# rasd3/TODA

Hardware: AMD Instinct MI355X
Metric: LiDAR training samples/sec (higher is better)
Workload: dtype f32

## Files before the change

toda_amd/csrc/rulebook.hip:

```cpp
#include "grid_index.cuh"
#include "scan.cuh"

namespace toda {

constexpr int RB_BLOCK = GI_TILE;

__global__ void __launch_bounds__(RB_BLOCK)
gi_mark_coords_kernel(const int4* __restrict__ idx, int n, const int32_t* __restrict__ n_dev, GridDims g,
                      uint2* __restrict__ cells) {
    n = eff_n(n, n_dev);
    const int i = blockIdx.x * RB_BLOCK + threadIdx.x;
    if (i >= n) return;
    const int4 c = idx[i];
    if (!in_grid(c, g)) return;
    gi_set_bit_first(cells, lin_index(c.x, c.y, c.z, c.w, g));
}

__global__ void __launch_bounds__(RB_BLOCK)
gi_rowof_kernel(const int4* __restrict__ idx, int n, const int32_t* __restrict__ n_dev, GridDims g,
                const uint2* __restrict__ cells, int* __restrict__ rowof) {
    n = eff_n(n, n_dev);
    const int i = blockIdx.x * RB_BLOCK + threadIdx.x;
    if (i >= n) return;
    const int4 c = idx[i];
// ... 332 lines not shown
    pairs_open(s_cnt, K);
    const int i = blockIdx.x * RB_BLOCK + threadIdx.x;
    const bool live = i < n_in;
    int4 c = make_int4(0, 0, 0, 0);
    if (live) c = idx[i];
    const bool inside = live && (unsigned)c.x < (unsigned)cg.out.B;
    int zo[KZ], yo[KY], xo[KX];
#pragma unroll
    for (int a = 0; a < KZ; ++a) zo[a] = out_coord(c.y, a, cg.st[0], cg.pd[0], cg.out.D);
#pragma unroll
    for (int a = 0; a < KY; ++a) yo[a] = out_coord(c.z, a, cg.st[1], cg.pd[1], cg.out.H);
#pragma unroll
    for (int a = 0; a < KX; ++a) xo[a] = out_coord(c.w, a, cg.st[2], cg.pd[2], cg.out.W);
    uint2 cell[K];
    unsigned bit[K];
#pragma unroll
    for (int k = 0; k < K; ++k) {
        const Tap t = tap_of<KY, KX>(k);
        cell[k] = make_uint2(0u, 0u);
        bit[k] = 0u;
        if (inside && zo[t.z] >= 0 && yo[t.y] >= 0 && xo[t.x] >= 0) gi_fetch(cells, lin_index(c.x, zo[t.z], yo[t.y], xo[t.x], cg.out), cell[k], bit[k]);
    }
#pragma unroll
    for (int k = 0; k < K; ++k) {
        int o = gi_rank_of(cell[k], bit[k]);
        if (o >= n_out) o = -1;
        if (o >= 0 && o2i) o2i[(size_t)k * n_out + o] = i;
        if (live) i2o[(size_t)k * n_in + i] = o;
        count_pairs(o >= 0, k, s_cnt);
    }
    pairs_flush(s_cnt, K, pair_cnt);
}

template <int KZ, int KY, int KX>
__global__ void __launch_bounds__(RB_BLOCK)
rb_conv_o2i_kernel(const int4* __restrict__ idx_out, int n_out, ConvGeom cg, GridDims gin, const uint2* __restrict__ cells_in,
                   const int* __restrict__ rowof_in, int n_in, int* __restrict__ o2i) {
    constexpr int K = KZ * KY * KX;
    const int o = blockIdx.x * RB_BLOCK + threadIdx.x;
    if (o >= n_out) return;
    const int4 c = idx_out[o];
    uint2 cell[K];
    unsigned bit[K];
#pragma unroll
    for (int k = 0; k < K; ++k) {
        const Tap t = tap_of<KY, KX>(k);
        cell[k] = make_uint2(0u, 0u);
        bit[k] = 0u;
        const int z = in_coord(c.y, t.z, cg.st[0], cg.pd[0]), y = in_coord(c.z, t.y, cg.st[1], cg.pd[1]), x = in_coord(c.w, t.x, cg.st[2], cg.pd[2]);
        if (in_grid(make_int4(c.x, z, y, x), gin)) gi_fetch(cells_in, lin_index(c.x, z, y, x, gin), cell[k], bit[k]);
    }
    int r[K];
#pragma unroll
    for (int k = 0; k < K; ++k) {
        r[k] = gi_rank_of(cell[k], bit[k]);
        if (r[k] >= n_in) r[k] = -1;
    }
    if (rowof_in) {
#pragma unroll
        for (int k = 0; k < K; ++k)
            if (r[k] >= 0) r[k] = rowof_in[r[k]];
    }
#pragma unroll
    for (int k = 0; k < K; ++k) o2i[(size_t)k * n_out + o] = r[k];
}

// ... 3 lines not shown
    __shared__ int s_cnt[64];
    pairs_open(s_cnt, 64);
    const int i = blockIdx.x * RB_BLOCK + threadIdx.x;
    const bool live = i < n_in;
    int4 c = make_int4(0, 0, 0, 0);
    if (live) c = idx[i];
    const bool inside = live && (unsigned)c.x < (unsigned)cg.out.B;
    int k = 0;
    for (int kz = 0; kz < cg.ks[0]; ++kz) {
        const int zo = out_coord(c.y, kz, cg.st[0], cg.pd[0], cg.out.D);
        for (int ky = 0; ky < cg.ks[1]; ++ky) {
            const int yo = out_coord(c.z, ky, cg.st[1], cg.pd[1], cg.out.H);
            for (int kx = 0; kx < cg.ks[2]; ++kx, ++k) {
                const int xo = out_coord(c.w, kx, cg.st[2], cg.pd[2], cg.out.W);
                uint2 cell = {};
                unsigned bit = 0u;
                if (inside && zo >= 0 && yo >= 0 && xo >= 0) gi_fetch(cells, lin_index(c.x, zo, yo, xo, cg.out), cell, bit);
                int o = gi_rank_of(cell, bit);
                if (o >= n_out) o = -1;
                if (o >= 0) o2i[(size_t)k * n_out + o] = i;
                if (live) i2o[(size_t)k * n_in + i] = o;
                count_pairs(o >= 0, k, s_cnt);
            }
        }
    }
    pairs_flush(s_cnt, k, pair_cnt);
}

struct ConvKernels {
    decltype(&rb_conv_generic_kernel) i2o;
    decltype(&rb_conv_o2i_kernel<3, 3, 3>) o2i;
};

static ConvKernels conv_kernels(const int32_t* ks) {
    if (ks[0] == 3 && ks[1] == 3 && ks[2] == 3) return {rb_conv_kernel<3, 3, 3>, rb_conv_o2i_kernel<3, 3, 3>};
    if (ks[0] == 3 && ks[1] == 1 && ks[2] == 1) return {rb_conv_kernel<3, 1, 1>, rb_conv_o2i_kernel<3, 1, 1>};
    return {rb_conv_generic_kernel, nullptr};
}

static int conv_setup(const char* who, int batch, const int32_t* shape_in, const int32_t* ks, const int32_t* st, const int32_t* pd,
                      const int32_t* shape_out, const void* gi_out, GiView* out, ConvGeom* cg) {
    int rc = gi_view(who, gi_out, batch, shape_out, out);
    if (rc) return rc;
    for (int a = 0; a < 3; ++a) {
        TODA_CHECK_ARG(ks[a] >= 1 && st[a] >= 1 && pd[a] >= 0, "%s: bad kernel/stride/pad on axis %d", who, a);
        TODA_CHECK_ARG(shape_in[a] + 2 * pd[a] >= ks[a], "%s: axis %d of %d cells (+ 2 * %d) is shorter than the kernel's %d", who, a,
                       shape_in[a], pd[a], ks[a]);
        const int expect = (shape_in[a] + 2 * pd[a] - ks[a]) / st[a] + 1;
        TODA_CHECK_ARG(shape_out[a] == expect, "%s: shape_out[%d]=%d but (in+2p-k)/s+1=%d", who, a, shape_out[a], expect);
        cg->ks[a] = ks[a];
        cg->st[a] = st[a];
        cg->pd[a] = pd[a];
    }
    TODA_CHECK_ARG(ks[0] * ks[1] * ks[2] <= 64, "%s: kernel volume > 64 unsupported", who);
    cg->out = out->dims;
    return TODA_OK;
}

}

using namespace toda;

extern "C" size_t toda_gridindex_bytes(int batch, const int32_t* shape_host) {
    return gi_layout(batch, shape_host).bytes;
}

extern "C" int toda_gridindex_from_coords(const int32_t* idx, int n, const int32_t* n_dev, int batch,
                                          const int32_t* shape_host, void* gi, int32_t* rowof, void* stream) {
// ... 101 lines not shown
    GiView v;
    int rc = gi_view("rulebook_subm", gi, batch, shape_host, &v);
    if (rc) return rc;
    const int K = ksize_host[0] * ksize_host[1] * ksize_host[2];
    TODA_CHECK_ARG(K >= 1 && K <= 64, "rulebook_subm: kernel volume %d unsupported", K);
    for (int a = 0; a < 3; ++a)
        TODA_CHECK_ARG(ksize_host[a] % 2 == 1 && dilation_host[a] >= 1, "rulebook_subm: kernel must be odd, dilation >= 1");
    if (!cnt_zeroed) TODA_HIP(hipMemsetAsync(pair_cnt, 0, K * sizeof(int32_t), s));
    if (n == 0) return TODA_OK;
    const uint2* cells = v.cells;
    const dim3 grid(cdiv(n, RB_BLOCK)), block(RB_BLOCK);
    if (ksize_host[0] == 3 && ksize_host[1] == 3 && ksize_host[2] == 3)
        hipLaunchKernelGGL(HIP_KERNEL_NAME(rb_subm_kernel<3, 3, 3>), grid, block, 0, s, (const int4*)idx, n, v.dims,
                           dilation_host[0], dilation_host[1], dilation_host[2], cells, rowof, nbr, pair_cnt);
    else
        hipLaunchKernelGGL(rb_subm_generic_kernel, grid, block, 0, s, (const int4*)idx, n, v.dims, ksize_host[0],
                           ksize_host[1], ksize_host[2], dilation_host[0], dilation_host[1], dilation_host[2], cells,
                           rowof, nbr, pair_cnt);
    TODA_LAUNCH_CHECK();
    return TODA_OK;
}

extern "C" int toda_rulebook_conv(const int32_t* idx_in, int n_in, int batch, const int32_t* shape_in_host,
                                  const int32_t* ksize_host, const int32_t* stride_host, const int32_t* pad_host,
                                  const int32_t* shape_out_host, const void* gi_out, int n_out, int32_t* nbr_o2i,
                                  int32_t* nbr_i2o, int32_t* pair_cnt, const int32_t* idx_out, const void* gi_in,
                                  const int32_t* rowof_in, int cnt_zeroed, void* stream) {
    hipStream_t s = (hipStream_t)stream;
    GiView out;
    ConvGeom cg;
    int rc = conv_setup("rulebook_conv", batch, shape_in_host, ksize_host, stride_host, pad_host, shape_out_host, gi_out, &out, &cg);
    if (rc) return rc;
    const int K = ksize_host[0] * ksize_host[1] * ksize_host[2];
    const ConvKernels kernels = conv_kernels(ksize_host);
    const bool by_output = idx_out && gi_in && kernels.o2i;
    if (!cnt_zeroed) TODA_HIP(hipMemsetAsync(pair_cnt, 0, K * sizeof(int32_t), s));
    if (n_out > 0 && !by_output) TODA_HIP(hipMemsetAsync(nbr_o2i, 0xFF, (size_t)K * n_out * sizeof(int32_t), s));
    const dim3 block(RB_BLOCK);
    if (by_output && n_out > 0) {
        GiView in;
        rc = gi_view("rulebook_conv", gi_in, batch, shape_in_host, &in);
        if (rc) return rc;
        hipLaunchKernelGGL(kernels.o2i, dim3(cdiv(n_out, RB_BLOCK)), block, 0, s, (const int4*)idx_out, n_out, cg, in.dims,
                           (const uint2*)in.cells, rowof_in, n_in, nbr_o2i);
    }
    if (n_in > 0)
        hipLaunchKernelGGL(kernels.i2o, dim3(cdiv(n_in, RB_BLOCK)), block, 0, s, (const int4*)idx_in, n_in, cg, (const uint2*)out.cells,
                           n_out, by_output ? nullptr : nbr_o2i, nbr_i2o, pair_cnt);
    TODA_LAUNCH_CHECK();
    return TODA_OK;
}
```

toda_amd/csrc/spconv.hip:

```cpp
#include <stdlib.h>

#include <type_traits>

#include <hip/hip_ext.h>

#include <mutex>
#include <vector>

#include "bn_fold.cuh"
#include "common.h"


namespace toda {

typedef float f32x4 __attribute__((ext_vector_type(4)));

constexpr int SC_BLOCK = 256;

static int tiles_pow2(int channels) {
    int t = (channels + 15) / 16, p = 1;
    while (p < t) p <<= 1;
    return p;
}

// ... 213 lines not shown
                to = qo[done + lane];
            }
            __builtin_amdgcn_wave_barrier();
            if (lane < left) {
                qi[lane] = ti;
                qo[lane] = to;
            }
        }
        qn = left;
        __builtin_amdgcn_wave_barrier();
    }
    if (qn > 0) round(0, qn, std::false_type{});
}

template <bool BOUND, int MTB, int NTB>
__device__ __forceinline__ void wg_store_slab(const f32x4 (&acc)[MTB][NTB], float* slab, int chunk, int k, int K, int MT, int NT,
                                              int m0, int n0, int cin, int cout, int ii, int g) {
    float* dst = slab + (size_t)chunk * cout * K * cin;
#pragma unroll
    for (int m = 0; m < MTB; ++m)
#pragma unroll
        for (int n = 0; n < NTB; ++n)
#pragma unroll
            for (int reg = 0; reg < 4; ++reg) {
                const int ci = MT * (4 * g + reg) + m0 + m;
                const int co = NT * ii + n0 + n;
                if (!BOUND || (ci < cin && co < cout)) dst[((size_t)co * K + k) * cin + ci] = acc[m][n][reg];
            }
}

struct GatherClasses {
    unsigned char count[8];
    unsigned char k[8][27];
};

template <int Q, int NT, int RT, bool VEC, bool CLS = false>
__global__ void __launch_bounds__(SC_BLOCK)
gather_gemm_kernel(const float* __restrict__ in, int n_in, int cg, const float* __restrict__ wp,
                   const int* __restrict__ nbr, int n_out, int K, int cp, const float* __restrict__ bias,
                   float* __restrict__ out, const int* __restrict__ order,
                   const unsigned char* __restrict__ cls_sorted, const GatherClasses classes) {
    const int lane = threadIdx.x & 63;
    const int wave = (int)blockIdx.x * (SC_BLOCK / 64) + (threadIdx.x >> 6);
    const int r = lane & 15, g = lane >> 4;
    const int row0 = wave * (16 * RT);
    if (row0 >= n_out) return;

    f32x4 acc[RT][NT];
#pragma unroll
    for (int n = 0; n < NT; ++n) {
        float b = 0.0f;
        if (bias && NT * r + n < cp) b = bias[NT * r + n];
#pragma unroll
        for (int rt = 0; rt < RT; ++rt) acc[rt][n] = f32x4{b, b, b, b};
    }
    const f32x4* __restrict__ wp4 = reinterpret_cast<const f32x4*>(wp);
    const __amdgpu_buffer_rsrc_t in_rsrc = table_rsrc(in, (unsigned)n_in * (unsigned)cg * 4u);
    int rows[RT];
    bool live[RT];
#pragma unroll
    for (int rt = 0; rt < RT; ++rt) {
        live[rt] = row0 + rt * 16 + r < n_out;
        rows[rt] = live[rt] ? (order ? order[row0 + rt * 16 + r] : row0 + rt * 16 + r) : n_out - 1;
    }

    auto load_ids = [&](int k, int (&dst)[RT]) {
// ... 731 lines not shown
    for (int s = 0; s < n; ++s) {
        TODA_CHECK_ARG(w[s] && wp[s] && cout[s] >= 1 && cin[s] >= 1 && k_vol[s] >= 1, "pack_weights: bad segment %d", s);
        const int cgather = transpose[s] ? cout[s] : cin[s], cprod = transpose[s] ? cin[s] : cout[s];
        TODA_CHECK_ARG(cgather <= 128 && cprod <= 128, "pack_weights: channels > 128 unsupported (segment %d)", s);
        if (use_split(cgather, cprod)) {
            split_pack_fill(sb, sm, w[s], cout[s], k_vol[s], cin[s], transpose[s], flip_k[s], wp[s]);
            const long long total = (long long)k_vol[s] * sb.KC[sm] * sb.NT[sm] * 192;
            if (total > smost) smost = total;
            if (++sm == toda::SPLIT_PACK_MAX_SEG) {
                const int rc = sflush();
                if (rc != TODA_OK) return rc;
            }
            continue;
        }
        const int i = m;
        b.w[i] = w[s], b.wp[i] = wp[s], b.cout[i] = cout[s], b.K[i] = k_vol[s], b.cin[i] = cin[s];
        b.transpose[i] = transpose[s] != 0, b.flip[i] = flip_k[s] != 0;
        b.Q[i] = (unsigned char)tiles_pow2(cgather), b.NT[i] = (unsigned char)tiles_pow2(cprod);
        const long long total = (long long)k_vol[s] * b.Q[i] * b.NT[i] * 256;
        if (total > most) most = total;
        if (++m == PACK_MAX_SEG) {
            const int rc = flush();
            if (rc != TODA_OK) return rc;
        }
    }
    {
        const int rc = flush();
        if (rc != TODA_OK) return rc;
    }
    return sflush();
}

namespace toda {
constexpr int CLS_ROWS = 8192, CLS_PER = CLS_ROWS / 256;
struct ClassGeom {
    int stride[3], pad[3];
};
__global__ void __launch_bounds__(256)
class_order_kernel(const int4* __restrict__ coords, int n, const ClassGeom gm, int32_t* __restrict__ order, unsigned char* __restrict__ cls_sorted) {
    __shared__ int cnt[8][256 + 1];
    const int base = blockIdx.x * CLS_ROWS, t = threadIdx.x;
    unsigned char c[CLS_PER];
    int mine[8] = {0, 0, 0, 0, 0, 0, 0, 0};
#pragma unroll
    for (int i = 0; i < CLS_PER; ++i) {
        const int r = base + t * CLS_PER + i;
        int cl = 0;
        if (r < n) {
            const int4 v = coords[r];
            cl = (((v.y + gm.pad[0]) % gm.stride[0]) * gm.stride[1] + (v.z + gm.pad[1]) % gm.stride[1]) * gm.stride[2] + (v.w + gm.pad[2]) % gm.stride[2];
            ++mine[cl & 7];
        }
        c[i] = (unsigned char)cl;
    }
#pragma unroll
    for (int k = 0; k < 8; ++k) cnt[k][t] = mine[k];
    __syncthreads();
    if (t < 8) {
        int run = 0;
        for (int j = 0; j < 256; ++j) {
            const int v = cnt[t][j];
            cnt[t][j] = run;
            run += v;
        }
        cnt[t][256] = run;
    }
    __syncthreads();
    int cls_base[8], run = 0;
#pragma unroll
    for (int k = 0; k < 8; ++k) {
        cls_base[k] = run + cnt[k][t];
        run += cnt[k][256];
    }
#pragma unroll
    for (int i = 0; i < CLS_PER; ++i) {
        const int r = base + t * CLS_PER + i;
        if (r >= n) break;
        const int k = c[i] & 7;
        int pos = 0;
#pragma unroll
        for (int q = 0; q < 8; ++q)
            if (q == k) pos = cls_base[q]++;
        order[base + pos] = r;
        cls_sorted[base + pos] = c[i];
    }
}

static int class_table(const int32_t* ksize, const int32_t* stride, const int32_t* pad, GatherClasses* out) {
    const int n_class = stride[0] * stride[1] * stride[2];
    if (n_class < 1 || n_class > 8 || ksize[0] * ksize[1] * ksize[2] > 27) return -1;
    *out = GatherClasses{};
    for (int rz = 0; rz < stride[0]; ++rz)
        for (int ry = 0; ry < stride[1]; ++ry)
            for (int rx = 0; rx < stride[2]; ++rx) {
                const int c = (rz * stride[1] + ry) * stride[2] + rx;
                int m = 0;
                for (int kz = 0; kz < ksize[0]; ++kz)
                    for (int ky = 0; ky < ksize[1]; ++ky)
                        for (int kx = 0; kx < ksize[2]; ++kx)
                            if (kz % stride[0] == rz && ky % stride[1] == ry && kx % stride[2] == rx)
                                out->k[c][m++] = (unsigned char)((kz * ksize[1] + ky) * ksize[2] + kx);
                out->count[c] = (unsigned char)m;
            }
    return 0;
}
}

extern "C" int toda_rulebook_class_order(const int32_t* in_coords, int n_in, const int32_t* stride, const int32_t* padding, int32_t* order,
                                         unsigned char* cls_sorted, void* stream) {
    TODA_CHECK_ARG(in_coords && stride && padding && order && cls_sorted && n_in >= 0, "rulebook_class_order: null argument");
    ClassGeom gm;
    for (int a = 0; a < 3; ++a) {
        TODA_CHECK_ARG(stride[a] >= 1 && stride[a] <= 2 && padding[a] >= 0, "rulebook_class_order: stride 1 or 2 per axis (got %d)", stride[a]);
        gm.stride[a] = stride[a], gm.pad[a] = padding[a];
    }
    if (n_in == 0) return TODA_OK;
    hipLaunchKernelGGL(class_order_kernel, dim3(cdiv(n_in, CLS_ROWS)), dim3(256), 0, (hipStream_t)stream, (const int4*)in_coords, n_in, gm, order,
                       cls_sorted);
    TODA_LAUNCH_CHECK();
    return TODA_OK;
}

namespace toda {
struct LaunchTimer {
    std::vector<hipEvent_t> ev;
    int used = 0;
    bool on = false;
};
static LaunchTimer g_timer;
static std::mutex g_timer_mu;
static inline void timer_next(hipEvent_t* start, hipEvent_t* stop) {
    *start = *stop = nullptr;
    if (!g_timer.on) return;
    std::lock_guard<std::mutex> lock(g_timer_mu);
    if (!g_timer.on || 2 * (g_timer.used + 1) > (int)g_timer.ev.size()) return;
    *start = g_timer.ev[2 * g_timer.used];
    *stop = g_timer.ev[2 * g_timer.used + 1];
    g_timer.used++;
}
}

#define GG_LAUNCH(kernel, grid, block, shmem, stream, ...)                                              \
    do {                                                                                               \
        hipEvent_t t0_, t1_;                                                                           \
        toda::timer_next(&t0_, &t1_);                                                                  \
        hipExtLaunchKernelGGL(kernel, grid, block, shmem, stream, t0_, t1_, 0, __VA_ARGS__);           \
    } while (0)

extern "C" int toda_timing_begin(int capacity) {
    TODA_CHECK_ARG(capacity > 0 && capacity <= (1 << 20), "timing_begin: capacity in (0, 2^20]");
// ... 331 lines not shown
```

toda_amd/csrc/spconv_split.cuh:

```cuda
#pragma once
#include "split_common.cuh"

namespace toda {

#ifndef WGS_ACCS
#define WGS_ACCS 2
#endif
#ifndef SP_STAMPS
#define SP_STAMPS 0
#endif
#if SP_STAMPS
#define SP_STAMP(i)                                                                               \
    do {                                                                                          \
        unsigned long long t_;                                                                    \
        __builtin_amdgcn_sched_barrier(0);                                                        \
        asm volatile("s_memtime %0\n\ts_waitcnt lgkmcnt(0)" : "=s"(t_)::"memory");                \
        __builtin_amdgcn_sched_barrier(0);                                                        \
        seg[i] += t_ - t_prev;                                                                    \
        t_prev = t_;                                                                              \
    } while (0)
#else
#define SP_STAMP(i)
#endif
#ifndef SP_ABLATE
// ... 72 lines not shown
        } else {
            if (gch < cout && pch < cin) x = w[((size_t)gch * K + kk) * cin + pch];
        }
        v[j] = sp_plane_of(x, plane);
    }
    b.wps[sg][e] = u32x4{(unsigned)v[0] | ((unsigned)v[1] << 16), (unsigned)v[2] | ((unsigned)v[3] << 16), (unsigned)v[4] | ((unsigned)v[5] << 16),
                         (unsigned)v[6] | ((unsigned)v[7] << 16)};
}

template <int KC, int NT, int WAVES, bool IL = false>
__global__ void __launch_bounds__(SC_BLOCK, WAVES)
gg_split_kernel(const float* __restrict__ in, int n_in, const u32x4* __restrict__ wps, const int* __restrict__ nbr, int n_out, int K, int cp,
                const float* __restrict__ bias, float* __restrict__ out, const int* __restrict__ order, double* __restrict__ stats,
                const unsigned char* __restrict__ cls_sorted, const GatherClasses classes) {
    constexpr int RT = 2;
    constexpr int CG = 32 * KC;
    constexpr int UNITS = NT * 3;
    constexpr int SLICE = UNITS * 64;
    static_assert(2 * SLICE * 16 >= (SC_BLOCK / 64) * 2 * 16 * NT * 4, "the statistics scratch aliases the weight buffers");
    __shared__ u32x4 wl[2 * SLICE];
    const int lane = threadIdx.x & 63, wv = threadIdx.x >> 6;
    const int blk = xcd_chunked_block(blockIdx.x, gridDim.x);
    const int wave = blk * (SC_BLOCK / 64) + wv;
    const int r = lane & 15, g = lane >> 4;
    const int row0 = wave * (16 * RT);

    f32x4 acc[RT][NT];
    int rows[RT];
    bool live[RT];
    gg_prologue<RT, NT>(bias, cp, row0, n_out, order, r, acc, rows, live);
    const __amdgpu_buffer_rsrc_t in_rsrc = table_rsrc(in, (unsigned)n_in * (unsigned)CG * 4u);
    int KE = K;
    bool listed = false;
    unsigned long long kpack = 0;
    if (cls_sorted) {
        const int p = row0 + (lane & (16 * RT - 1));
        const int c = cls_sorted[p < n_out ? p : n_out - 1], c0 = __builtin_amdgcn_readfirstlane(c);
        const bool same = __all(c == c0 || p >= n_out);
        int* cw = reinterpret_cast<int*>(wl);
        if (lane == 0) cw[wv] = same ? c0 : -1;
        __syncthreads();
        int cb = cw[0];
#pragma unroll
        for (int w = 1; w < SC_BLOCK / 64; ++w) cb = (cw[w] == cb) ? cb : -1;
        __syncthreads();
        if (cb >= 0 && classes.count[cb & 7] > 0 && classes.count[cb & 7] <= 8) {
            listed = true;
            KE = classes.count[cb & 7];
#pragma unroll
            for (int i = 0; i < 8; ++i) kpack |= (unsigned long long)classes.k[cb & 7][i] << (8 * i);
            kpack = ((unsigned long long)__builtin_amdgcn_readfirstlane((int)(kpack >> 32)) << 32) | (unsigned)__builtin_amdgcn_readfirstlane((int)kpack);
        }
    }
    auto kof = [&](int j) { return listed ? (int)((kpack >> (8 * j)) & 0xFF) : j; };
    auto load_ids = [&](int j, int (&dst)[RT]) {
        const int kk = kof(j < KE ? j : KE - 1);
#pragma unroll
        for (int rt = 0; rt < RT; ++rt) {
            dst[rt] = __builtin_nontemporal_load(nbr + (size_t)kk * n_out + rows[rt]);
        }
    };
    auto gather_rt = [&](const int (&src)[RT], int part, bool valid, f32x4 (&raw)[RT][2], int rt) {
        const bool ok = src[rt] >= 0 && valid;
        const unsigned base = (unsigned)src[rt] * (unsigned)(CG * 4) + (unsigned)(16 * g) + 128u * (unsigned)part;
#pragma unroll
        for (int i = 0; i < 2; ++i)
            raw[rt][i] = __builtin_bit_cast(f32x4, __builtin_amdgcn_raw_buffer_load_b128(in_rsrc, ok ? base + 64u * i : OOB, 0, 0));
    };
    auto gather = [&](const int (&src)[RT], int part, bool valid, f32x4 (&raw)[RT][2]) {
#pragma unroll
        for (int rt = 0; rt < RT; ++rt) gather_rt(src, part, valid, raw, rt);
    };
    auto stage = [&](int st, int buf) {
        const int sc = st < KE * KC ? st : KE * KC - 1;
        const int ss = kof(sc / KC) * KC + sc % KC;
#pragma unroll
        for (int t = 0; t < (UNITS + SC_BLOCK / 64 - 1) / (SC_BLOCK / 64); ++t) {
            const int u = t * (SC_BLOCK / 64) + wv;
            if (UNITS % (SC_BLOCK / 64) == 0 || u < UNITS)
                __builtin_amdgcn_global_load_lds(reinterpret_cast<const float*>(wps + (size_t)ss * SLICE + u * 64 + lane),
                                                 reinterpret_cast<float*>(&wl[buf * SLICE + u * 64]), 16, 0, 0);
        }
    };

    int idA[RT], idB[RT], idC[RT];
    f32x4 raw[RT][2];
    load_ids(0, idA);
// ... 286 lines not shown
```

toda_amd/csrc/conv2d.hip:

```cpp
#include <hip/hip_ext.h>
#include <stdlib.h>
#include <string.h>

#include <algorithm>

#include "common.h"

#ifndef TODA_ABLATE
#define TODA_ABLATE 0
#endif

namespace toda {

typedef float f32x4 __attribute__((ext_vector_type(4)));
typedef float f32x2 __attribute__((ext_vector_type(2)));
typedef unsigned int u32x4w __attribute__((ext_vector_type(4)));

constexpr int WN_BLOCK = 256;
constexpr int WN_TILES = 32;
constexpr int WN_COUT = 32;
constexpr int WN_KC = 8;
constexpr int WN_FREQ = 36;
constexpr int WN_IMG = 256;
constexpr unsigned WN_OOB = 0xFFFFFFF0u;
// ... 77 lines not shown

__global__ void __launch_bounds__(WN_BLOCK)
wino_weight_kernel(const float* __restrict__ w, int cout, int cin, int mode, float* __restrict__ u) {
    wn_weight_element(w, cout, cin, mode, u, blockIdx.x * WN_BLOCK + threadIdx.x);
}

constexpr int WB_MAX_LAYERS = 16;
struct WeightBatch {
    const float* w[WB_MAX_LAYERS];
    float* u[WB_MAX_LAYERS];
    int cout[WB_MAX_LAYERS], cin[WB_MAX_LAYERS], mode[WB_MAX_LAYERS];
    unsigned first_block[WB_MAX_LAYERS + 1];
    int n;
};

__global__ void __launch_bounds__(WN_BLOCK)
wino_weight_batch_kernel(const WeightBatch b) {
    int l = 0;
    while (l + 1 < b.n && blockIdx.x >= b.first_block[l + 1]) ++l;
    wn_weight_element(b.w[l], b.cout[l], b.cin[l], b.mode[l], b.u[l], (blockIdx.x - b.first_block[l]) * WN_BLOCK + threadIdx.x);
}

__device__ __forceinline__ __amdgpu_buffer_rsrc_t wn_rsrc(const float* base, unsigned bytes) {
    return __builtin_amdgcn_make_buffer_rsrc(const_cast<float*>(base), 0, bytes, 0x00020000);
}

__device__ __forceinline__ int wn_work_id() {
    const int nwg = gridDim.x, xcd = blockIdx.x & 7, q8 = nwg >> 3, r8 = nwg & 7;
    return (xcd < r8 ? xcd * (q8 + 1) : r8 * (q8 + 1) + (xcd - r8) * q8) + (blockIdx.x >> 3);
}

struct PatchOff {
    unsigned offc[6];
    unsigned offe[6];
    bool left, right;
    bool tail;
};

__device__ __forceinline__ PatchOff wn_patch_off(int tile, int t, int chan, int C, const WinoGeom& g) {
    PatchOff p;
    const bool exists = tile < g.n_tiles;
    const int tl = exists ? tile : 0;
    const int b = tl / g.tiles_img, rem = tl - b * g.tiles_img;
    const int ty = rem / g.tiles_x, tx = rem - ty * g.tiles_x;
    const int y0 = 4 * ty, x0 = 4 * tx;
    const int base = ((b * C + chan) * g.H + (y0 - 1)) * g.W + x0;
    const bool has_l = x0 > 0, has_r = x0 + 4 < g.W;
    p.left = has_l || t == 0;
    p.right = has_r || t == 15;
    p.tail = x0 + 3 >= g.W;
#pragma unroll
    for (int r = 0; r < 6; ++r) {
        const int yy = y0 - 1 + r;
        const bool rv = exists && yy >= 0 && yy < g.H;
        const int row = base + r * g.W;
        p.offc[r] = rv ? (unsigned)row * 4u : WN_OOB;
        p.offe[r] = (rv && t == 0 && has_l) ? (unsigned)(row - 1) * 4u : (rv && t == 15 && has_r) ? (unsigned)(row + 4) * 4u : WN_OOB;
    }
    return p;
}

struct Patch {
    f32x2 p[6], q[6], e[6];
};

__device__ __forceinline__ float wn_dpp_from_prev(float own, float v) {
    return __builtin_bit_cast(float, __builtin_amdgcn_update_dpp(__builtin_bit_cast(int, own), __builtin_bit_cast(int, v), 0x111, 0xF, 0xF, false));
}
__device__ __forceinline__ float wn_dpp_from_next(float own, float v) {
    return __builtin_bit_cast(float, __builtin_amdgcn_update_dpp(__builtin_bit_cast(int, own), __builtin_bit_cast(int, v), 0x101, 0xF, 0xF, false));
}

__device__ __forceinline__ void wn_load_patch(__amdgpu_buffer_rsrc_t rsrc, const PatchOff& o, unsigned soff, Patch& d) {
#pragma unroll
    for (int r = 0; r < 6; ++r) {
        const f32x4 c = __builtin_bit_cast(f32x4, __builtin_amdgcn_raw_buffer_load_b128(rsrc, o.offc[r], soff, 0));
        const float e = __builtin_bit_cast(float, __builtin_amdgcn_raw_buffer_load_b32(rsrc, o.offe[r], soff, 0));
        const float l = wn_dpp_from_prev(e, c[3]), rr = wn_dpp_from_next(e, c[0]);
        d.p[r] = f32x2{c[0], c[1]};
        d.q[r] = f32x2{o.tail ? 0.0f : c[2], o.tail ? 0.0f : c[3]};
        d.e[r] = f32x2{o.left ? l : 0.0f, o.right ? rr : 0.0f};
    }
}

struct PatchRaw {
    f32x4 c[6];
    float e[6];
    bool left, right, tail;
};

__device__ __forceinline__ void wn_load_raw(__amdgpu_buffer_rsrc_t rsrc, const PatchOff& o, unsigned soff, PatchRaw& d) {
#pragma unroll
    for (int r = 0; r < 6; ++r) {
        d.c[r] = __builtin_bit_cast(f32x4, __builtin_amdgcn_raw_buffer_load_b128(rsrc, o.offc[r], soff, 0));
        d.e[r] = __builtin_bit_cast(float, __builtin_amdgcn_raw_buffer_load_b32(rsrc, o.offe[r], soff, 0));
    }
    d.left = o.left, d.right = o.right, d.tail = o.tail;
}

__device__ __forceinline__ void wn_finish_patch(const PatchRaw& s, Patch& d) {
#pragma unroll
    for (int r = 0; r < 6; ++r) {
        const float l = wn_dpp_from_prev(s.e[r], s.c[r][3]), rr = wn_dpp_from_next(s.e[r], s.c[r][0]);
        d.p[r] = f32x2{s.c[r][0], s.c[r][1]};
        d.q[r] = f32x2{s.tail ? 0.0f : s.c[r][2], s.tail ? 0.0f : s.c[r][3]};
        d.e[r] = f32x2{s.left ? l : 0.0f, s.right ? rr : 0.0f};
    }
}

__device__ __forceinline__ f32x2 wn_fma2(float c, f32x2 a, f32x2 b) {
    return __builtin_elementwise_fma(f32x2{c, c}, a, b);
}

__device__ __forceinline__ void wn_bt2(const f32x2 (&d)[6], f32x2 (&v)[6]) {
    const f32x2 a = d[3] - d[1], b = d[4] - d[2];
    v[0] = wn_fma2(1.5f, a, wn_fma2(-2.0f, d[2], d[0] + d[4]));
    v[1] = wn_fma2(-2.5f, d[2], wn_fma2(0.5f, d[3], d[1] + d[4]));
    v[2] = wn_fma2(2.5f, d[3], wn_fma2(0.5f, d[2], d[4] - d[1]));
    v[3] = wn_fma2(2.0f, a, b);
    v[4] = wn_fma2(-0.5f, a, b);
    v[5] = wn_fma2(1.5f, b, wn_fma2(-2.0f, d[3], d[1] + d[5]));
}

__device__ __forceinline__ f32x2 w2_lo(f32x2 a) { return __builtin_shufflevector(a, a, 0, 0); }
__device__ __forceinline__ f32x2 w2_hi(f32x2 a) { return __builtin_shufflevector(a, a, 1, 1); }
__device__ __forceinline__ f32x2 w2_fma(f32x2 a, f32x2 b, f32x2 c) { return __builtin_elementwise_fma(a, b, c); }
#define W2_K(a_, b_) ((unsigned long long)__builtin_bit_cast(unsigned, (float)(a_)) | ((unsigned long long)__builtin_bit_cast(unsigned, (float)(b_)) << 32))
#define W2_KK(a_) W2_K(a_, a_)
__device__ __forceinline__ f32x2 w2_add(f32x2 a, f32x2 b) {
    f32x2 d;
    asm("v_pk_add_f32 %0, %1, %2" : "=v"(d) : "v"(a), "v"(b));
    return d;
}
__device__ __forceinline__ f32x2 w2_sub(f32x2 a, f32x2 b) {
    f32x2 d;
    asm("v_pk_add_f32 %0, %1, %2 neg_lo:[0,1] neg_hi:[0,1]" : "=v"(d) : "v"(a), "v"(b));
    return d;
}
__device__ __forceinline__ f32x2 w2_mul(f32x2 a, f32x2 b) {
    f32x2 d;
// ... 337 lines not shown
                }
            } else if (!(ablate & 4)) wn_input_transform_store(d, lds + buf * IMG + a_off);
            else lds[buf * IMG + a_off] = d.p[0][0] + d.e[5][1] + d.q[2][0];
        };

        WinoCursor ld = ws_cursor(lo, g.n_chunks, true);
        PatchOff pa = patch_of(ld.unit);
        const unsigned x_bytes = (unsigned)((size_t)g.B * g.Cin * g.H * g.W * 4u), u_bytes = (unsigned)((size_t)WN_FREQ * g.Cin * g.Cout * 4u);
        const unsigned u_voff = (unsigned)pt * 16u;
        auto fetch = [&](Stage& st, int q_fetch) {
            const bool live = q_fetch < total;
            const __amdgpu_buffer_rsrc_t xr_q = wn_rsrc(x, live && !(ablate & 1) ? x_bytes : 0u);
            const __amdgpu_buffer_rsrc_t ur_q = wn_rsrc(u, live && !(ablate & 2) ? u_bytes : 0u);
            wn_load_raw(xr_q, pa, (unsigned)ld.chunk * chunk_bytes, st.d);
            const unsigned u_soff = (unsigned)((cb_of(ld.unit) * g.n_chunks + ld.chunk) * IMG) * 4u;
#pragma unroll
            for (int it = 0; it < B_IT; ++it)
                st.b[it] = __builtin_bit_cast(f32x4, __builtin_amdgcn_raw_buffer_load_b128(ur_q, u_voff, u_soff + (unsigned)it * 4096u, 0));
            if (live) {
                if (++ld.chunk == g.n_chunks) {
                    ld.chunk = 0;
                    ld.unit += 1;
                    if (q_fetch + 1 < total && (gang || ld.unit % g.n_cout_blocks == 0)) pa = patch_of(ld.unit);
                }
            }
        };
        wn_produce_stream<Stage>(total, fetch, produce);
    }
}

constexpr int WG_KT = 8;
constexpr int WG_SLAB_FLOATS = WN_FREQ * 32 * 32;

struct TilePos {
    int b, ty, tx;
    bool exists;
};

__device__ __forceinline__ TilePos wn_tile_pos(int tile, const WinoGeom& g) {
    TilePos t;
    t.exists = tile < g.n_tiles;
    const int tl = t.exists ? tile : 0;
    t.b = tl / g.tiles_img;
    const int rem = tl - t.b * g.tiles_img;
    t.ty = rem / g.tiles_x;
    t.tx = rem - t.ty * g.tiles_x;
    return t;
}

__device__ __forceinline__ void wn_tile_advance(TilePos& t, int step, int tile_after, const WinoGeom& g) {
    t.tx += step;
    while (t.tx >= g.tiles_x) {
        t.tx -= g.tiles_x;
        if (++t.ty == g.tiles_y) {
            t.ty = 0;
            ++t.b;
        }
    }
    t.exists = tile_after < g.n_tiles;
}

__device__ __forceinline__ float wn_quad_from_prev(float own, float v) {
    const float s = __builtin_bit_cast(float, __builtin_amdgcn_update_dpp(0, __builtin_bit_cast(int, v), 0x90, 0xF, 0xF, false));
    return (threadIdx.x & 3) == 0 ? own : s;
}
__device__ __forceinline__ float wn_quad_from_next(float own, float v) {
// ... 79 lines not shown
        asm("v_pk_fma_f32 %0, %1, %2, %1 op_sel:[1,0,0] op_sel_hi:[1,1,0]" : "=v"(u) : "v"(P), "s"(W2_K(0.5f, -2.0f)));
        asm("v_pk_fma_f32 %0, %1, %2, %0 op_sel:[0,0,0] op_sel_hi:[0,1,1]" : "+v"(u) : "v"(Q), "s"(W2_K(0.25f, 4.0f)));
        asm("v_pk_fma_f32 %0, %1, %2, %0 op_sel:[1,0,0] op_sel_hi:[1,1,1]" : "+v"(u) : "v"(Q), "s"(W2_K(0.125f, -8.0f)));
        dst[(i * 6 + 0) * WN_IMG] = P[0];
        dst[(i * 6 + 1) * WN_IMG] = m12[0];
        dst[(i * 6 + 2) * WN_IMG] = m12[1];
        dst[(i * 6 + 3) * WN_IMG] = u[0];
        dst[(i * 6 + 4) * WN_IMG] = u[1];
        dst[(i * 6 + 5) * WN_IMG] = Q[1];
    }
}

struct WgradGeom {
    WinoGeom g;
    int n_ci_blocks, n_co_blocks, n_units, steps_per_unit;
};

__global__ void __launch_bounds__(WS_BLOCK, 2)
wino_wgrad_kernel(const float* __restrict__ x, const float* __restrict__ dy, const WgradGeom wg, float* __restrict__ slabs, const int ablate_arg) {
    const int ablate = TODA_ABLATE ? ablate_arg : 0;
    __shared__ float lds[4 * WN_FREQ * WN_IMG];
    constexpr int IMG = WN_FREQ * WN_IMG;
    const WinoGeom& g = wg.g;
    const int tid = threadIdx.x, lane = tid & 63, wave = tid >> 6;
    const int G = gridDim.x;
    const int w = wn_work_id();
    const long long S = (long long)wg.n_units * wg.steps_per_unit;
    const long long lo = ws_range_lo(w, G, S), hi = ws_range_lo(w + 1, G, S);
    const int total = __builtin_amdgcn_readfirstlane((int)(hi - lo));
    if (total == 0) return;

    if (wave < 4) {
        const int wm = wave >> 1, wn = wave & 1;
        const f32x2* const a_frag = reinterpret_cast<const f32x2*>(lds) + wm * 64 + lane;
        const f32x2* const b_frag = reinterpret_cast<const f32x2*>(lds + 2 * IMG) + wn * 64 + lane;
        int q = 0;
        long long s = lo;
        while (s < hi) {
            const WinoCursor at = ws_cursor(s, wg.steps_per_unit);
            const int unit = at.unit, c_begin = at.chunk, c_end = ws_segment_end(s, hi, c_begin, wg.steps_per_unit);
            f32x4 acc[WN_FREQ];
#pragma unroll
            for (int f = 0; f < WN_FREQ; ++f) acc[f] = f32x4{0.f, 0.f, 0.f, 0.f};
            for (int chunk = c_begin; chunk < c_end; ++chunk, ++q) {
                __syncthreads();
                wn_consume_chunk(acc, a_frag + (q & 1) * (IMG / 2), b_frag + (q & 1) * (IMG / 2), ablate);
            }
            s += c_end - c_begin;
            float* const sl = slabs + (size_t)(w + unit) * WG_SLAB_FLOATS + (wn * 16 + (lane & 15)) * 32 + wm * 16 + (lane >> 4) * 4;
#pragma unroll
            for (int f = 0; f < WN_FREQ; ++f) *reinterpret_cast<f32x4*>(sl + f * 1024) = acc[f];
        }
    } else {
        const int pw = wave - 4;
        const int k = (lane & 3) + 4 * (pw & 1), slot = (lane >> 2) + 16 * (pw >> 1);
        const int img_off = (slot >> 4) * 128 + ((k >> 1) * 16 + (slot & 15)) * 2 + (k & 1);
        const WinoCursor first = ws_cursor(lo, wg.steps_per_unit, true);
        int unit = first.unit, chunk = first.chunk;
        TilePos tp = wn_tile_pos(chunk * WG_KT + k, g);
        const unsigned x_bytes = (unsigned)((size_t)g.B * g.Cin * g.H * g.W * 4u), y_bytes = (unsigned)((size_t)g.B * g.Cout * g.H * g.W * 4u);

        struct WStage {
            XRaw x;
            DyRaw y;
        };
        auto fetch = [&](WStage& st, int q_fetch) {
            const bool live = q_fetch < total;
            const __amdgpu_buffer_rsrc_t xr = wn_rsrc(x, live && !(ablate & 1) ? x_bytes : 0u), yr = wn_rsrc(dy, live && !(ablate & 2) ? y_bytes : 0u);
            const int cib = unit / wg.n_co_blocks, cob = unit - cib * wg.n_co_blocks;
            wn_load_x(xr, tp, cib * 32 + slot, g, st.x);
            wn_load_dy(yr, tp, cob * 32 + slot, g, st.y);
            if (live) {
                if (++chunk == wg.steps_per_unit) {
                    chunk = 0;
                    ++unit;
                    tp = wn_tile_pos(k, g);
                } else {
                    wn_tile_advance(tp, WG_KT, chunk * WG_KT + k, g);
                }
            }
        };
        auto produce = [&](const WStage& st, int buf) {
            if (ablate & 4) {
                float* const d0 = lds + buf * IMG + img_off;
                float* const d1 = lds + (2 + buf) * IMG + img_off;
#pragma unroll
                for (int f = 0; f < WN_FREQ; ++f) {
                    d0[f * WN_IMG] = st.x.c[f % 6][f & 3];
                    d1[f * WN_IMG] = st.y.c[f & 3][f % 4];
// ... 323 lines not shown
```

Before: 150.2.

## Add parity-class stride-2 rulebook kernel, wave-ballot class sort, union-class tap lists

Adds a specialized rulebook kernel for 3x3x3 stride-2 convolutions that uses input-coordinate parity to fetch at most 8 candidate output cells instead of 27, sharing a bitmap word when two lookups land in the same word. The class-ordering kernel is rewritten to use 1024 threads with wave ballots and a shuffle-based scan in place of a serial per-class scan. The gather-GEMM now handles blocks with mixed parity classes by taking the union of their tap sets from a per-class bitmask, so more blocks can skip the taps that are absent for them. These changes cut hash probes and empty-tap work, at the cost of more complex index logic and possible extra register pressure.

```diff
diff --git a/toda_amd/csrc/rulebook.hip b/toda_amd/csrc/rulebook.hip
--- a/toda_amd/csrc/rulebook.hip
+++ b/toda_amd/csrc/rulebook.hip
@@ -388,6 +388,61 @@
     pairs_flush(s_cnt, K, pair_cnt);
 }
 
+__global__ void __launch_bounds__(RB_BLOCK)
+rb_conv_s2_kernel(const int4* __restrict__ idx, int n_in, ConvGeom cg, const uint2* __restrict__ cells, int n_out,
+                  int* __restrict__ o2i, int* __restrict__ i2o, int* __restrict__ pair_cnt) {
+    constexpr int K = 27;
+    __shared__ int s_cnt[K];
+    pairs_open(s_cnt, K);
+    const int i = blockIdx.x * RB_BLOCK + threadIdx.x;
+    const bool live = i < n_in;
+    int4 c = make_int4(0, 0, 0, 0);
+    if (live) c = idx[i];
+    const bool inside = live && (unsigned)c.x < (unsigned)cg.out.B;
+    const int pz = (c.y + cg.pd[0]) & 1, py = (c.z + cg.pd[1]) & 1, px = (c.w + cg.pd[2]) & 1;
+    int zo[2], yo[2], xo[2];
+#pragma unroll
+    for (int j = 0; j < 2; ++j) {
+        zo[j] = (j == 0 || pz == 0) ? out_coord(c.y, 2 * j + pz, 2, cg.pd[0], cg.out.D) : -1;
+        yo[j] = (j == 0 || py == 0) ? out_coord(c.z, 2 * j + py, 2, cg.pd[1], cg.out.H) : -1;
+        xo[j] = (j == 0 || px == 0) ? out_coord(c.w, 2 * j + px, 2, cg.pd[2], cg.out.W) : -1;
+    }
+    uint2 cell[8];
+    unsigned bit[8];
+    bool same_word[4];
+#pragma unroll
+    for (int jzy = 0; jzy < 4; ++jzy) {
+        const int z = zo[jzy >> 1], y = yo[jzy & 1];
+        const bool row = inside && z >= 0 && y >= 0;
+        const long long l0 = lin_index(c.x, z, y, xo[0], cg.out), l1 = lin_index(c.x, z, y, xo[1], cg.out);
+        const bool ok0 = row && xo[0] >= 0, ok1 = row && xo[1] >= 0;
+        same_word[jzy] = ok0 && ok1 && (l0 >> 5) == (l1 >> 5);
+        cell[2 * jzy] = cell[2 * jzy + 1] = make_uint2(0u, 0u);
+        bit[2 * jzy] = bit[2 * jzy + 1] = 0u;
+        if (ok0) gi_fetch(cells, l0, cell[2 * jzy], bit[2 * jzy]);
+        if (ok1 && !same_word[jzy]) gi_fetch(cells, l1, cell[2 * jzy + 1], bit[2 * jzy + 1]);
+        if (same_word[jzy]) bit[2 * jzy + 1] = 1u << (l1 & 31);
+    }
+    int res[8];
+#pragma unroll
+    for (int j = 0; j < 8; ++j) {
+        const uint2 w = (j & 1) && same_word[j >> 1] ? cell[j - 1] : cell[j];
+        res[j] = gi_rank_of(w, bit[j]);
+        if (res[j] >= n_out) res[j] = -1;
+    }
+    const int cls = (pz * 2 + py) * 2 + px;
+#pragma unroll
+    for (int k = 0; k < K; ++k) {
+        const Tap t = tap_of<3, 3>(k);
+        int o = -1;
+        if (cls == (((t.z & 1) * 2 + (t.y & 1)) * 2 + (t.x & 1))) o = res[((t.z >> 1) * 2 + (t.y >> 1)) * 2 + (t.x >> 1)];
+        if (o >= 0 && o2i) o2i[(size_t)k * n_out + o] = i;
+        if (live) i2o[(size_t)k * n_in + i] = o;
+        count_pairs(o >= 0, k, s_cnt);
+    }
+    pairs_flush(s_cnt, K, pair_cnt);
+}
+
 template <int KZ, int KY, int KX>
 __global__ void __launch_bounds__(RB_BLOCK)
 rb_conv_o2i_kernel(const int4* __restrict__ idx_out, int n_out, ConvGeom cg, GridDims gin, const uint2* __restrict__ cells_in,
@@ -457,8 +512,9 @@
     decltype(&rb_conv_o2i_kernel<3, 3, 3>) o2i;
 };
 
-static ConvKernels conv_kernels(const int32_t* ks) {
-    if (ks[0] == 3 && ks[1] == 3 && ks[2] == 3) return {rb_conv_kernel<3, 3, 3>, rb_conv_o2i_kernel<3, 3, 3>};
+static ConvKernels conv_kernels(const int32_t* ks, const int32_t* st) {
+    if (ks[0] == 3 && ks[1] == 3 && ks[2] == 3)
+        return {st[0] == 2 && st[1] == 2 && st[2] == 2 ? rb_conv_s2_kernel : rb_conv_kernel<3, 3, 3>, rb_conv_o2i_kernel<3, 3, 3>};
     if (ks[0] == 3 && ks[1] == 1 && ks[2] == 1) return {rb_conv_kernel<3, 1, 1>, rb_conv_o2i_kernel<3, 1, 1>};
     return {rb_conv_generic_kernel, nullptr};
 }
@@ -626,7 +682,7 @@
     int rc = conv_setup("rulebook_conv", batch, shape_in_host, ksize_host, stride_host, pad_host, shape_out_host, gi_out, &out, &cg);
     if (rc) return rc;
     const int K = ksize_host[0] * ksize_host[1] * ksize_host[2];
-    const ConvKernels kernels = conv_kernels(ksize_host);
+    const ConvKernels kernels = conv_kernels(ksize_host, stride_host);
     const bool by_output = idx_out && gi_in && kernels.o2i;
     if (!cnt_zeroed) TODA_HIP(hipMemsetAsync(pair_cnt, 0, K * sizeof(int32_t), s));
     if (n_out > 0 && !by_output) TODA_HIP(hipMemsetAsync(nbr_o2i, 0xFF, (size_t)K * n_out * sizeof(int32_t), s));
diff --git a/toda_amd/csrc/spconv.hip b/toda_amd/csrc/spconv.hip
--- a/toda_amd/csrc/spconv.hip
+++ b/toda_amd/csrc/spconv.hip
@@ -269,6 +269,7 @@
 struct GatherClasses {
     unsigned char count[8];
     unsigned char k[8][27];
+    unsigned int bits[8];
 };
 
 template <int Q, int NT, int RT, bool VEC, bool CLS = false>
@@ -1066,57 +1067,61 @@
 }
 
 namespace toda {
-constexpr int CLS_ROWS = 8192, CLS_PER = CLS_ROWS / 256;
+constexpr int CLS_ROWS = 8192, CLS_THREADS = 1024, CLS_PER = CLS_ROWS / CLS_THREADS, CLS_TILES = CLS_ROWS / 64;
+static_assert(8 * CLS_TILES == CLS_THREADS, "one thread per (class, tile) counter in the scan");
 struct ClassGeom {
     int stride[3], pad[3];
 };
-__global__ void __launch_bounds__(256)
+__device__ __forceinline__ int cls_mod(int x, int s) {
+    const int m = x & (s - 1);
+    return (x < 0 && m) ? m - s : m;
+}
+__global__ void __launch_bounds__(CLS_THREADS)
 class_order_kernel(const int4* __restrict__ coords, int n, const ClassGeom gm, int32_t* __restrict__ order, unsigned char* __restrict__ cls_sorted) {
-    __shared__ int cnt[8][256 + 1];
-    const int base = blockIdx.x * CLS_ROWS, t = threadIdx.x;
-    unsigned char c[CLS_PER];
-    int mine[8] = {0, 0, 0, 0, 0, 0, 0, 0};
+    __shared__ int cnt[8 * CLS_TILES];
+    __shared__ int wsum[CLS_THREADS / 64];
+    const int base = blockIdx.x * CLS_ROWS, t = threadIdx.x, lane = t & 63, wv = t >> 6;
+    int4 v[CLS_PER];
 #pragma unroll
     for (int i = 0; i < CLS_PER; ++i) {
-        const int r = base + t * CLS_PER + i;
-        int cl = 0;
-        if (r < n) {
-            const int4 v = coords[r];
-            cl = (((v.y + gm.pad[0]) % gm.stride[0]) * gm.stride[1] + (v.z + gm.pad[1]) % gm.stride[1]) * gm.stride[2] + (v.w + gm.pad[2]) % gm.stride[2];
-            ++mine[cl & 7];
-        }
-        c[i] = (unsigned char)cl;
-    }
-#pragma unroll
-    for (int k = 0; k < 8; ++k) cnt[k][t] = mine[k];
+        const int r = base + i * CLS_THREADS + t;
+        v[i] = make_int4(0, 0, 0, 0);
+        if (r < n) v[i] = coords[r];
+    }
+    int key[CLS_PER];
+#pragma unroll
+    for (int i = 0; i < CLS_PER; ++i) {
+        const bool live = base + i * CLS_THREADS + t < n;
+        const int cl = (cls_mod(v[i].y + gm.pad[0], gm.stride[0]) * gm.stride[1] + cls_mod(v[i].z + gm.pad[1], gm.stride[1])) * gm.stride[2] +
+                       cls_mod(v[i].w + gm.pad[2], gm.stride[2]);
+        const unsigned long long lv = __ballot(live), b0 = __ballot((cl & 1) != 0), b1 = __ballot((cl & 2) != 0), b2 = __ballot((cl & 4) != 0);
+        auto lanes_of = [&](int q) { return lv & ((q & 1) ? b0 : ~b0) & ((q & 2) ? b1 : ~b1) & ((q & 4) ? b2 : ~b2); };
+        const unsigned long long same = lanes_of(cl);
+        const int rank = __builtin_amdgcn_mbcnt_hi((unsigned)(same >> 32), __builtin_amdgcn_mbcnt_lo((unsigned)same, 0u));
+        if (lane < 8) cnt[lane * CLS_TILES + i * (CLS_THREADS / 64) + wv] = __popcll(lanes_of(lane));
+        key[i] = (cl & 0xFF) | (rank << 8);
+    }
     __syncthreads();
-    if (t < 8) {
-        int run = 0;
-        for (int j = 0; j < 256; ++j) {
-            const int v = cnt[t][j];
-            cnt[t][j] = run;
-            run += v;
-        }
-        cnt[t][256] = run;
-    }
+    const int mine = cnt[t];
+    int incl = mine;
+#pragma unroll
+    for (int d = 1; d < 64; d <<= 1) {
+        const int up = __shfl_up(incl, d, 64);
+        if (lane >= d) incl += up;
+    }
+    if (lane == 63) wsum[wv] = incl;
     __syncthreads();
-    int cls_base[8], run = 0;
-#pragma unroll
-    for (int k = 0; k < 8; ++k) {
-        cls_base[k] = run + cnt[k][t];
-        run += cnt[k][256];
-    }
+    int before = 0;
+    for (int w = 0; w < wv; ++w) before += wsum[w];
+    cnt[t] = before + incl - mine;
+    __syncthreads();
 #pragma unroll
     for (int i = 0; i < CLS_PER; ++i) {
-        const int r = base + t * CLS_PER + i;
+        const int r = base + i * CLS_THREADS + t;
         if (r >= n) break;
-        const int k = c[i] & 7;
-        int pos = 0;
-#pragma unroll
-        for (int q = 0; q < 8; ++q)
-            if (q == k) pos = cls_base[q]++;
+        const int pos = cnt[(key[i] & 7) * CLS_TILES + i * (CLS_THREADS / 64) + wv] + (key[i] >> 8);
         order[base + pos] = r;
-        cls_sorted[base + pos] = c[i];
+        cls_sorted[base + pos] = (unsigned char)key[i];
     }
 }
 
@@ -1132,8 +1137,11 @@
                 for (int kz = 0; kz < ksize[0]; ++kz)
                     for (int ky = 0; ky < ksize[1]; ++ky)
                         for (int kx = 0; kx < ksize[2]; ++kx)
-                            if (kz % stride[0] == rz && ky % stride[1] == ry && kx % stride[2] == rx)
-                                out->k[c][m++] = (unsigned char)((kz * ksize[1] + ky) * ksize[2] + kx);
+                            if (kz % stride[0] == rz && ky % stride[1] == ry && kx % stride[2] == rx) {
+                                const int k = (kz * ksize[1] + ky) * ksize[2] + kx;
+                                out->k[c][m++] = (unsigned char)k;
+                                out->bits[c] |= 1u << k;
+                            }
                 out->count[c] = (unsigned char)m;
             }
     return 0;
@@ -1149,7 +1157,7 @@
         gm.stride[a] = stride[a], gm.pad[a] = padding[a];
     }
     if (n_in == 0) return TODA_OK;
-    hipLaunchKernelGGL(class_order_kernel, dim3(cdiv(n_in, CLS_ROWS)), dim3(256), 0, (hipStream_t)stream, (const int4*)in_coords, n_in, gm, order,
+    hipLaunchKernelGGL(class_order_kernel, dim3(cdiv(n_in, CLS_ROWS)), dim3(CLS_THREADS), 0, (hipStream_t)stream, (const int4*)in_coords, n_in, gm, order,
                        cls_sorted);
     TODA_LAUNCH_CHECK();
     return TODA_OK;
diff --git a/toda_amd/csrc/spconv_split.cuh b/toda_amd/csrc/spconv_split.cuh
--- a/toda_amd/csrc/spconv_split.cuh
+++ b/toda_amd/csrc/spconv_split.cuh
@@ -128,27 +128,47 @@
     const __amdgpu_buffer_rsrc_t in_rsrc = table_rsrc(in, (unsigned)n_in * (unsigned)CG * 4u);
     int KE = K;
     bool listed = false;
-    unsigned long long kpack = 0;
+    unsigned long long kpack[4] = {0, 0, 0, 0};
     if (cls_sorted) {
         const int p = row0 + (lane & (16 * RT - 1));
-        const int c = cls_sorted[p < n_out ? p : n_out - 1], c0 = __builtin_amdgcn_readfirstlane(c);
-        const bool same = __all(c == c0 || p >= n_out);
+        const int c = cls_sorted[p < n_out ? p : n_out - 1] & 7;
+        unsigned mine = 0;
+#pragma unroll
+        for (int q = 0; q < 8; ++q) mine |= (__ballot(c == q && p < n_out) != 0ull ? 1u : 0u) << q;
         int* cw = reinterpret_cast<int*>(wl);
-        if (lane == 0) cw[wv] = same ? c0 : -1;
+        if (lane == 0) cw[wv] = (int)mine;
         __syncthreads();
-        int cb = cw[0];
-#pragma unroll
-        for (int w = 1; w < SC_BLOCK / 64; ++w) cb = (cw[w] == cb) ? cb : -1;
+        unsigned cm = 0;
+#pragma unroll
+        for (int w = 0; w < SC_BLOCK / 64; ++w) cm |= (unsigned)cw[w];
         __syncthreads();
-        if (cb >= 0 && classes.count[cb & 7] > 0 && classes.count[cb & 7] <= 8) {
+        if (cm == 0) cm = 1u << c;
+        cm = (unsigned)__builtin_amdgcn_readfirstlane((int)cm);
+        unsigned kbits = 0;
+        bool known = true;
+#pragma unroll
+        for (int q = 0; q < 8; ++q)
+            if ((cm >> q) & 1u) {
+                kbits |= classes.bits[q];
+                known = known && classes.count[q] > 0;
+            }
+        if (known && kbits) {
             listed = true;
-            KE = classes.count[cb & 7];
-#pragma unroll
-            for (int i = 0; i < 8; ++i) kpack |= (unsigned long long)classes.k[cb & 7][i] << (8 * i);
-            kpack = ((unsigned long long)__builtin_amdgcn_readfirstlane((int)(kpack >> 32)) << 32) | (unsigned)__builtin_amdgcn_readfirstlane((int)kpack);
-        }
-    }
-    auto kof = [&](int j) { return listed ? (int)((kpack >> (8 * j)) & 0xFF) : j; };
+            KE = __popc(kbits);
+            unsigned rest = kbits;
+            for (int m = 0; rest; ++m, rest &= rest - 1) {
+                const unsigned long long e = (unsigned long long)__builtin_ctz(rest) << (8 * (m & 7));
+#pragma unroll
+                for (int h = 0; h < 4; ++h)
+                    if ((m >> 3) == h) kpack[h] |= e;
+            }
+        }
+    }
+    auto kof = [&](int j) {
+        if (!listed) return j;
+        const unsigned long long pk = j < 8 ? kpack[0] : j < 16 ? kpack[1] : j < 24 ? kpack[2] : kpack[3];
+        return (int)((pk >> (8 * (j & 7))) & 0xFF);
+    };
     auto load_ids = [&](int j, int (&dst)[RT]) {
         const int kk = kof(j < KE ? j : KE - 1);
 #pragma unroll
```

Result: no change. 151.0, median of 6 (+0.5%).

## Load one halo element per lane and swizzle wgrad LDS fragment layout

Applied to the files above, without the earlier changes.

Halo edge loading now issues a single 32-bit buffer load per lane instead of six. Lanes 0-5 and 8-13 of each 16-lane row fetch the left and right halo elements for the row's six patch rows, and DPP row shifts redistribute them to the edge lanes. This cuts redundant scattered loads and address registers, at the cost of extra DPP moves and more complex address math. Separately, the wgrad kernel XOR-swizzles the LDS fragment index on both the producer store and the consumer read, which is meant to reduce LDS bank conflicts.

```diff
diff --git a/toda_amd/csrc/conv2d.hip b/toda_amd/csrc/conv2d.hip
--- a/toda_amd/csrc/conv2d.hip
+++ b/toda_amd/csrc/conv2d.hip
@@ -133,7 +133,7 @@
 
 struct PatchOff {
     unsigned offc[6];
-    unsigned offe[6];
+    unsigned offe;
     bool left, right;
     bool tail;
 };
@@ -154,10 +154,16 @@
     for (int r = 0; r < 6; ++r) {
         const int yy = y0 - 1 + r;
         const bool rv = exists && yy >= 0 && yy < g.H;
-        const int row = base + r * g.W;
-        p.offc[r] = rv ? (unsigned)row * 4u : WN_OOB;
-        p.offe[r] = (rv && t == 0 && has_l) ? (unsigned)(row - 1) * 4u : (rv && t == 15 && has_r) ? (unsigned)(row + 4) * 4u : WN_OOB;
-    }
+        p.offc[r] = rv ? (unsigned)(base + r * g.W) * 4u : WN_OOB;
+    }
+    const bool side_r = t >= 8;
+    const int er = t & 7, etile = tile - t + (side_r ? 15 : 0);
+    const bool e_exists = er < 6 && etile < g.n_tiles;
+    const int el = e_exists ? etile : 0;
+    const int eb = el / g.tiles_img, erem = el - eb * g.tiles_img;
+    const int ety = erem / g.tiles_x, ex0 = 4 * (erem - ety * g.tiles_x);
+    const int eyy = 4 * ety - 1 + er, ex = side_r ? ex0 + 4 : ex0 - 1;
+    p.offe = (e_exists && eyy >= 0 && eyy < g.H && ex >= 0 && ex < g.W) ? (unsigned)(((eb * C + chan) * g.H + eyy) * g.W + ex) * 4u : WN_OOB;
     return p;
 }
 
@@ -172,41 +178,41 @@
     return __builtin_bit_cast(float, __builtin_amdgcn_update_dpp(__builtin_bit_cast(int, own), __builtin_bit_cast(int, v), 0x101, 0xF, 0xF, false));
 }
 
-__device__ __forceinline__ void wn_load_patch(__amdgpu_buffer_rsrc_t rsrc, const PatchOff& o, unsigned soff, Patch& d) {
-#pragma unroll
-    for (int r = 0; r < 6; ++r) {
-        const f32x4 c = __builtin_bit_cast(f32x4, __builtin_amdgcn_raw_buffer_load_b128(rsrc, o.offc[r], soff, 0));
-        const float e = __builtin_bit_cast(float, __builtin_amdgcn_raw_buffer_load_b32(rsrc, o.offe[r], soff, 0));
-        const float l = wn_dpp_from_prev(e, c[3]), rr = wn_dpp_from_next(e, c[0]);
-        d.p[r] = f32x2{c[0], c[1]};
-        d.q[r] = f32x2{o.tail ? 0.0f : c[2], o.tail ? 0.0f : c[3]};
-        d.e[r] = f32x2{o.left ? l : 0.0f, o.right ? rr : 0.0f};
-    }
-}
-
 struct PatchRaw {
     f32x4 c[6];
-    float e[6];
+    float e;
     bool left, right, tail;
 };
 
 __device__ __forceinline__ void wn_load_raw(__amdgpu_buffer_rsrc_t rsrc, const PatchOff& o, unsigned soff, PatchRaw& d) {
 #pragma unroll
+    for (int r = 0; r < 6; ++r) d.c[r] = __builtin_bit_cast(f32x4, __builtin_amdgcn_raw_buffer_load_b128(rsrc, o.offc[r], soff, 0));
+    d.e = __builtin_bit_cast(float, __builtin_amdgcn_raw_buffer_load_b32(rsrc, o.offe, soff, 0));
+    d.left = o.left, d.right = o.right, d.tail = o.tail;
+}
+
+template <int N>
+__device__ __forceinline__ float wn_dpp_row_shift(float v) {
+    if constexpr (N == 0) return v;
+    else return __builtin_bit_cast(float, __builtin_amdgcn_update_dpp(__builtin_bit_cast(int, v), __builtin_bit_cast(int, v), N > 0 ? 0x100 + N : 0x110 - N, 0xF, 0xF, false));
+}
+
+__device__ __forceinline__ void wn_finish_patch(const PatchRaw& s, Patch& d) {
+    const float el[6] = {s.e, wn_dpp_row_shift<1>(s.e), wn_dpp_row_shift<2>(s.e), wn_dpp_row_shift<3>(s.e), wn_dpp_row_shift<4>(s.e), wn_dpp_row_shift<5>(s.e)};
+    const float er[6] = {wn_dpp_row_shift<-7>(s.e), wn_dpp_row_shift<-6>(s.e), wn_dpp_row_shift<-5>(s.e), wn_dpp_row_shift<-4>(s.e), wn_dpp_row_shift<-3>(s.e), wn_dpp_row_shift<-2>(s.e)};
+#pragma unroll
     for (int r = 0; r < 6; ++r) {
-        d.c[r] = __builtin_bit_cast(f32x4, __builtin_amdgcn_raw_buffer_load_b128(rsrc, o.offc[r], soff, 0));
-        d.e[r] = __builtin_bit_cast(float, __builtin_amdgcn_raw_buffer_load_b32(rsrc, o.offe[r], soff, 0));
-    }
-    d.left = o.left, d.right = o.right, d.tail = o.tail;
-}
-
-__device__ __forceinline__ void wn_finish_patch(const PatchRaw& s, Patch& d) {
-#pragma unroll
-    for (int r = 0; r < 6; ++r) {
-        const float l = wn_dpp_from_prev(s.e[r], s.c[r][3]), rr = wn_dpp_from_next(s.e[r], s.c[r][0]);
+        const float l = wn_dpp_from_prev(el[r], s.c[r][3]), rr = wn_dpp_from_next(er[r], s.c[r][0]);
         d.p[r] = f32x2{s.c[r][0], s.c[r][1]};
         d.q[r] = f32x2{s.tail ? 0.0f : s.c[r][2], s.tail ? 0.0f : s.c[r][3]};
         d.e[r] = f32x2{s.left ? l : 0.0f, s.right ? rr : 0.0f};
     }
+}
+
+__device__ __forceinline__ void wn_load_patch(__amdgpu_buffer_rsrc_t rsrc, const PatchOff& o, unsigned soff, Patch& d) {
+    PatchRaw raw;
+    wn_load_raw(rsrc, o, soff, raw);
+    wn_finish_patch(raw, d);
 }
 
 __device__ __forceinline__ f32x2 wn_fma2(float c, f32x2 a, f32x2 b) {
@@ -610,6 +616,8 @@
 constexpr int WG_KT = 8;
 constexpr int WG_SLAB_FLOATS = WN_FREQ * 32 * 32;
 
+__device__ __forceinline__ int wg_swizzle(int slot8) { return slot8 ^ ((slot8 >> 1) & 8); }
+
 struct TilePos {
     int b, ty, tx;
     bool exists;
@@ -755,8 +763,8 @@
 
     if (wave < 4) {
         const int wm = wave >> 1, wn = wave & 1;
-        const f32x2* const a_frag = reinterpret_cast<const f32x2*>(lds) + wm * 64 + lane;
-        const f32x2* const b_frag = reinterpret_cast<const f32x2*>(lds + 2 * IMG) + wn * 64 + lane;
+        const f32x2* const a_frag = reinterpret_cast<const f32x2*>(lds) + wm * 64 + wg_swizzle(lane);
+        const f32x2* const b_frag = reinterpret_cast<const f32x2*>(lds + 2 * IMG) + wn * 64 + wg_swizzle(lane);
         int q = 0;
         long long s = lo;
         while (s < hi) {
@@ -777,7 +785,7 @@
     } else {
         const int pw = wave - 4;
         const int k = (lane & 3) + 4 * (pw & 1), slot = (lane >> 2) + 16 * (pw >> 1);
-        const int img_off = (slot >> 4) * 128 + ((k >> 1) * 16 + (slot & 15)) * 2 + (k & 1);
+        const int img_off = (slot >> 4) * 128 + wg_swizzle((k >> 1) * 16 + (slot & 15)) * 2 + (k & 1);
         const WinoCursor first = ws_cursor(lo, wg.steps_per_unit, true);
         int unit = first.unit, chunk = first.chunk;
         TilePos tp = wn_tile_pos(chunk * WG_KT + k, g);
```

Measured after the change: 150.0 before, 151.0 after, median of 6. About the same (+0.6%).
